# zhupan007/Detection_3D

Measured on AMD Instinct MI355X. Metric: buildings/sec inference, 4c_fpn432, higher is better.
Workload: dtype f32

## Files before the change

### detection_3d_amd/_lib.py

```python
import ctypes
import os

import torch

_HERE = os.path.dirname(os.path.abspath(__file__))
LIB_PATH = os.environ.get("D3D_LIB_PATH") or os.path.join(_HERE, "lib", "libd3d_hip.so")

_lib = None

c_int_p = ctypes.POINTER(ctypes.c_int)
c_float_p = ctypes.POINTER(ctypes.c_float)
vp = ctypes.c_void_p


class BnPrologue(ctypes.Structure):
    _fields_ = [("mean", vp), ("invstd", vp), ("weight", vp), ("bias", vp), ("leakiness", ctypes.c_float),
                ("out_stats", vp), ("out_stats_cap", ctypes.c_int), ("out_stats_rows", ctypes.POINTER(ctypes.c_int))]


bn_p = ctypes.POINTER(BnPrologue)

_SIGS = {
    "d3d_last_error": (ctypes.c_char_p, []),
    "d3d_abi_version": (ctypes.c_int, []),
    "d3d_meta_create": (ctypes.c_int, [ctypes.POINTER(vp), ctypes.c_size_t]),
    "d3d_meta_destroy": (ctypes.c_int, [vp]),
    "d3d_meta_clear": (ctypes.c_int, [vp]),
    "d3d_meta_arena_used": (ctypes.c_int, [vp, ctypes.POINTER(ctypes.c_size_t)]),
    "d3d_meta_set_geometry_stream": (ctypes.c_int, [vp, vp, ctypes.c_int]),
    "d3d_meta_set_plan_stream": (ctypes.c_int, [vp, vp, ctypes.c_int]),
    "d3d_geometry_async_start": (ctypes.c_int, [vp, vp, ctypes.c_int, vp, vp]),
    "d3d_geometry_async_wait": (ctypes.c_int, [vp, ctypes.c_int, ctypes.POINTER(ctypes.c_int), vp]),
    "d3d_geometry_async_finish": (ctypes.c_int, [vp]),
    "d3d_grid_chain_enable": (ctypes.c_int, [ctypes.c_int]),
    "d3d_conv_ws_mode": (ctypes.c_int, [ctypes.c_int]),
    "d3d_conv_late_mode": (ctypes.c_int, [ctypes.c_int]),
    "d3d_conv_dw_deterministic": (ctypes.c_int, [ctypes.c_int]),
    "d3d_conv_dw_thread_mode": (ctypes.c_int, [ctypes.c_int, vp, ctypes.c_size_t]),
    "d3d_conv_dw_scratch_bytes": (ctypes.c_size_t, [ctypes.c_int, ctypes.c_int, ctypes.c_int]),
    "d3d_grid_chain_head": (ctypes.c_int, [ctypes.c_int]),
    "d3d_sort_scratch_bytes": (ctypes.c_size_t, [ctypes.c_int, ctypes.c_int]),
    "d3d_sort_pairs": (ctypes.c_int, [vp, vp, ctypes.c_int, ctypes.c_int, ctypes.c_int, vp, vp, vp, ctypes.c_size_t, vp]),
    "d3d_conv_time_next": (ctypes.c_int, [vp, vp]),
    "d3d_input_layer_prepare": (ctypes.c_int, [vp, vp]),
    "d3d_post_scores": (ctypes.c_int, [vp, ctypes.c_int, ctypes.c_int, ctypes.c_float, vp, vp, vp]),
    "d3d_post_order": (ctypes.c_int, [vp, ctypes.c_int, ctypes.c_int, vp, vp]),
    "d3d_post_gather": (ctypes.c_int, [vp, vp, ctypes.c_int, ctypes.c_int, vp, vp, vp, vp]),
    "d3d_post_select_max": (ctypes.c_int, []),
    "d3d_post_select": (ctypes.c_int, [vp, vp, ctypes.c_int, ctypes.c_int, vp, vp, ctypes.c_int, ctypes.c_int, vp, vp, vp, vp,
                                       vp]),
    "d3d_roi_prepare": (ctypes.c_int, [vp, ctypes.c_int, ctypes.c_float, c_float_p, ctypes.c_int, ctypes.c_float, vp, vp,
                                       vp, vp]),
    "d3d_roi_prepare_counted": (ctypes.c_int, [vp, ctypes.c_int, vp, ctypes.c_float, c_float_p, ctypes.c_int,
                                               ctypes.c_float, vp, vp, vp, vp]),
    "d3d_voxelize": (ctypes.c_int, [vp, ctypes.c_int, ctypes.c_int, ctypes.c_double, c_int_p, vp, vp,
                                    c_int_p, vp, ctypes.c_size_t, vp]),
    "d3d_voxelize_scratch_bytes": (ctypes.c_size_t, [ctypes.c_int]),
    "d3d_input_layer_build": (ctypes.c_int, [vp, vp, ctypes.c_int, ctypes.c_int, c_int_p, ctypes.c_int,
                                             ctypes.c_int, vp, c_int_p]),
    "d3d_input_layer_build_prefetch": (ctypes.c_int, [vp, vp, ctypes.c_int, ctypes.c_int, c_int_p, ctypes.c_int,
                                                      ctypes.c_int, c_int_p, vp, c_int_p]),
    "d3d_input_layer_forward": (ctypes.c_int, [vp, vp, ctypes.c_int, vp, vp]),
    "d3d_input_layer_export": (ctypes.c_int, [vp, vp, vp, vp]),
    "d3d_get_n_active": (ctypes.c_int, [vp, c_int_p, c_int_p]),
    "d3d_get_spatial_locations": (ctypes.c_int, [vp, c_int_p, vp, vp]),
    "d3d_subm_prepare": (ctypes.c_int, [vp, c_int_p, c_int_p, vp, ctypes.POINTER(ctypes.c_long)]),
    "d3d_conv_prepare": (ctypes.c_int, [vp, c_int_p, c_int_p, c_int_p, c_int_p, vp, c_int_p,
                                        ctypes.POINTER(ctypes.c_long)]),
    "d3d_deconv_prepare": (ctypes.c_int, [vp, c_int_p, c_int_p, c_int_p, c_int_p, vp,
                                          ctypes.POINTER(ctypes.c_long)]),
    "d3d_export_rules": (ctypes.c_int, [vp, ctypes.c_int, c_int_p, c_int_p, c_int_p, vp, ctypes.c_long,
                                        ctypes.POINTER(ctypes.c_long), vp]),
    "d3d_packed_weight_floats": (ctypes.c_size_t, [ctypes.c_int, ctypes.c_int, ctypes.c_int]),
    "d3d_pack_conv_weight": (ctypes.c_int, [vp, ctypes.c_int, ctypes.c_int, ctypes.c_int, vp, vp]),
    "d3d_subm_conv_forward": (ctypes.c_int, [vp, c_int_p, c_int_p, vp, ctypes.c_int, vp, ctypes.c_int, vp,
                                             vp, vp, ctypes.POINTER(ctypes.c_double), bn_p]),
    "d3d_conv_forward": (ctypes.c_int, [vp, c_int_p, c_int_p, c_int_p, c_int_p, vp, ctypes.c_int, vp,
                                        ctypes.c_int, vp, vp, ctypes.POINTER(ctypes.c_double), bn_p]),
    "d3d_deconv_forward": (ctypes.c_int, [vp, c_int_p, c_int_p, c_int_p, c_int_p, vp, ctypes.c_int, vp,
                                          ctypes.c_int, vp, vp, vp, ctypes.POINTER(ctypes.c_double), bn_p]),
    "d3d_bn_apply": (ctypes.c_int, [vp, vp, ctypes.c_int, ctypes.c_int, vp, vp, vp, vp, ctypes.c_float, vp]),
    "d3d_bn_batch_invstd": (ctypes.c_int, [vp, ctypes.c_int, ctypes.c_int, ctypes.c_float, vp, vp, vp,
                                           ctypes.c_size_t, vp]),
    "d3d_pack_conv_weight_transposed": (ctypes.c_int, [vp, ctypes.c_int, ctypes.c_int, ctypes.c_int, ctypes.c_int,
                                                       vp, vp]),
    "d3d_subm_conv_backward": (ctypes.c_int, [vp, c_int_p, c_int_p, vp, ctypes.c_int, vp, ctypes.c_int, vp, vp,
                                              vp, vp]),
    "d3d_conv_backward": (ctypes.c_int, [vp, c_int_p, c_int_p, c_int_p, c_int_p, vp, ctypes.c_int, vp,
                                         ctypes.c_int, vp, vp, vp, vp]),
    "d3d_deconv_backward": (ctypes.c_int, [vp, c_int_p, c_int_p, c_int_p, c_int_p, vp, ctypes.c_int, vp,
                                           ctypes.c_int, vp, vp, vp, vp]),
    "d3d_bn_backward": (ctypes.c_int, [vp, vp, vp, vp, ctypes.c_int, ctypes.c_int, vp, vp, vp, vp, vp,
                                       ctypes.c_float, vp, ctypes.c_size_t, vp]),
    "d3d_bn_backward_scratch_bytes": (ctypes.c_size_t, [ctypes.c_int]),
    "d3d_input_layer_backward": (ctypes.c_int, [vp, vp, ctypes.c_int, vp, vp]),
    "d3d_sparse_to_dense_backward": (ctypes.c_int, [vp, c_int_p, vp, ctypes.c_int, vp, vp]),
    "d3d_roi_align_rotated_3d_backward": (ctypes.c_int, [vp, ctypes.c_int, ctypes.c_int, ctypes.c_int, ctypes.c_int,
                                                         ctypes.c_int, vp, ctypes.c_int, ctypes.c_float,
                                                         ctypes.c_int, ctypes.c_int, ctypes.c_int, ctypes.c_int,
                                                         vp, vp]),
    "d3d_roi_align_rotated_3d_sparse_backward": (ctypes.c_int, [vp, c_int_p, vp, ctypes.c_int, c_int_p, vp,
                                                                ctypes.c_int, ctypes.c_float, ctypes.c_int,
                                                                ctypes.c_int, ctypes.c_int, ctypes.c_int,
                                                                vp, vp]),
    "d3d_roi_align_rotated_3d_sparse_backward_deterministic": (
        ctypes.c_int, [vp, c_int_p, vp, ctypes.c_int, c_int_p, vp, ctypes.c_int, ctypes.c_float, ctypes.c_int,
                       ctypes.c_int, ctypes.c_int, ctypes.c_int, vp, ctypes.c_int, vp, ctypes.c_size_t, vp]),
    "d3d_roi_align_rotated_3d_sparse_backward_deterministic_scratch_bytes": (
        ctypes.c_size_t, [ctypes.c_int, ctypes.c_int, ctypes.c_int, ctypes.c_int, ctypes.c_int, ctypes.c_int,
                          ctypes.c_int]),
    "d3d_bn_forward": (ctypes.c_int, [vp, vp, ctypes.c_int, ctypes.c_int, vp, vp, vp, vp, vp, vp,
                                      ctypes.c_float, ctypes.c_float, ctypes.c_int, ctypes.c_float, vp,
                                      ctypes.c_size_t, vp]),
    "d3d_bn_batch_stats": (ctypes.c_int, [vp, ctypes.c_int, ctypes.c_int, vp, vp, vp, ctypes.c_size_t, vp]),
    "d3d_bn_scratch_bytes": (ctypes.c_size_t, [ctypes.c_int]),
    "d3d_add": (ctypes.c_int, [vp, vp, vp, ctypes.c_size_t, vp]),
    "d3d_sparse_to_dense_forward": (ctypes.c_int, [vp, c_int_p, vp, ctypes.c_int, ctypes.c_int, vp, vp]),
    "d3d_roi_align_rotated_3d_forward": (ctypes.c_int, [vp, ctypes.c_int, ctypes.c_int, ctypes.c_int,
                                                        ctypes.c_int, ctypes.c_int, vp, ctypes.c_int,
                                                        ctypes.c_float, ctypes.c_int, ctypes.c_int,
                                                        ctypes.c_int, ctypes.c_int, vp, vp]),
    "d3d_roi_align_rotated_3d_sparse_forward": (ctypes.c_int, [vp, c_int_p, vp, ctypes.c_int, c_int_p, vp,
                                                               ctypes.c_int, ctypes.c_float, ctypes.c_int,
                                                               ctypes.c_int, ctypes.c_int, ctypes.c_int,
                                                               vp, ctypes.c_int, ctypes.c_int, vp, vp]),
    "d3d_roi_align_rotated_3d_sparse_forward_levels": (ctypes.c_int, [vp, ctypes.c_int, c_int_p, ctypes.POINTER(vp),
                                                                      ctypes.c_int, c_float_p, vp, ctypes.c_int,
                                                                      ctypes.c_int, ctypes.c_int, ctypes.c_int,
                                                                      ctypes.c_int, vp, ctypes.c_int, vp, vp]),
    "d3d_rotate_iou_eval": (ctypes.c_int, [vp, ctypes.c_int, vp, ctypes.c_int, ctypes.c_int, vp, vp]),
    "d3d_boxes_iou_3d": (ctypes.c_int, [vp, ctypes.c_int, vp, ctypes.c_int, ctypes.POINTER(ctypes.c_float),
                                        ctypes.c_int, ctypes.c_int, vp, vp]),
    "d3d_match_segments": (ctypes.c_int, [vp, c_int_p, ctypes.c_int, vp, ctypes.c_int, vp, ctypes.POINTER(ctypes.c_float),
                                          ctypes.c_int, ctypes.c_float, ctypes.c_float, ctypes.c_float, ctypes.c_int,
                                          ctypes.POINTER(ctypes.c_float), vp, vp, vp, ctypes.c_size_t, vp]),
    "d3d_match_segments_scratch_bytes": (ctypes.c_size_t, [ctypes.c_int, ctypes.c_int]),
    "d3d_rotate_nms_3d_batched": (ctypes.c_int, [vp, vp, ctypes.c_int, vp, ctypes.c_int, ctypes.c_int, ctypes.c_float,
                                                 ctypes.c_float, ctypes.c_float, ctypes.c_int, vp, vp, vp,
                                                 ctypes.c_size_t, vp]),
    "d3d_nms_batched_scratch_bytes": (ctypes.c_size_t, [ctypes.c_int, ctypes.c_int]),
    "d3d_rotate_nms_3d": (ctypes.c_int, [vp, vp, ctypes.c_int, ctypes.c_int, ctypes.c_int, ctypes.c_float, ctypes.c_float,
                                         ctypes.c_float, vp, vp, c_int_p, vp, ctypes.c_size_t, vp]),
    "d3d_rotate_nms_3d_scratch_bytes": (ctypes.c_size_t, [ctypes.c_int, ctypes.c_int]),
    "d3d_topk_segments": (ctypes.c_int, [vp, ctypes.c_int, ctypes.c_int, ctypes.c_int, ctypes.c_int, vp, ctypes.c_int,
                                         ctypes.c_int, ctypes.c_int, c_float_p, c_int_p, vp, ctypes.c_int, vp,
                                         ctypes.c_float, vp, vp, vp, vp, vp, vp, ctypes.c_size_t, vp]),
    "d3d_topk_scratch_bytes": (ctypes.c_size_t, [ctypes.c_int, ctypes.c_int]),
    "d3d_topk_max": (ctypes.c_int, []),
    "d3d_anchors": (ctypes.c_int, [vp, c_int_p, ctypes.POINTER(ctypes.c_float), ctypes.c_int,
                                   ctypes.POINTER(ctypes.c_float), ctypes.c_float, vp, vp]),
    "d3d_anchors_maps": (ctypes.c_int, [vp, ctypes.c_int, c_int_p, ctypes.POINTER(ctypes.c_float), ctypes.c_int,
                                        ctypes.POINTER(ctypes.c_float), ctypes.c_float, vp, vp]),
    "d3d_rpn_head": (ctypes.c_int, [ctypes.POINTER(vp), c_int_p, ctypes.c_int, ctypes.c_int, vp, vp, vp, vp,
                                    ctypes.c_int, vp, vp, vp]),
    "d3d_mlp_heads": (ctypes.c_int, [vp, ctypes.c_int, ctypes.c_int, ctypes.c_int, vp, vp, vp, vp, vp, ctypes.c_int, vp, vp, vp]),
    "d3d_rotate_nms_3d_sorted": (ctypes.c_int, [vp, ctypes.c_int, ctypes.c_float, ctypes.c_int, vp, vp, vp,
                                                ctypes.c_size_t, vp]),
    "d3d_nms_scratch_bytes": (ctypes.c_size_t, [ctypes.c_int]),
    "d3d_box_decode": (ctypes.c_int, [vp, vp, ctypes.c_int, ctypes.POINTER(ctypes.c_float), ctypes.c_float,
                                      vp, vp]),
    "d3d_box_decode_classes": (ctypes.c_int, [vp, vp, ctypes.c_int, ctypes.c_int, ctypes.POINTER(ctypes.c_float),
                                              ctypes.c_float, vp, vp]),
    "d3d_box_decode_rows": (ctypes.c_int, [vp, vp, vp, ctypes.c_int, ctypes.POINTER(ctypes.c_float), ctypes.c_float,
                                           vp, vp]),
    "d3d_gather_kept": (ctypes.c_int, [vp, vp, vp, vp, ctypes.c_int, ctypes.c_float, vp, vp, vp, vp]),
    "d3d_plan_stats": (ctypes.c_int, [vp, ctypes.c_int, c_int_p, c_int_p, c_int_p, ctypes.POINTER(ctypes.c_long),
                                      ctypes.POINTER(ctypes.c_long), ctypes.POINTER(ctypes.c_long), vp]),
    "d3d_packed_weight_bytes": (ctypes.c_size_t, [ctypes.c_int, ctypes.c_int, ctypes.c_int, ctypes.c_int]),
    "d3d_pack_conv_weight_dt": (ctypes.c_int, [vp, ctypes.c_int, ctypes.c_int, ctypes.c_int, vp, ctypes.c_int, vp]),
    "d3d_subm_conv_forward_dt": (ctypes.c_int, [vp, c_int_p, c_int_p, vp, ctypes.c_int, vp, ctypes.c_int, vp, vp,
                                                ctypes.c_int, vp, ctypes.POINTER(ctypes.c_double), bn_p]),
    "d3d_conv_forward_dt": (ctypes.c_int, [vp, c_int_p, c_int_p, c_int_p, c_int_p, vp, ctypes.c_int, vp, ctypes.c_int,
                                           vp, ctypes.c_int, vp, ctypes.POINTER(ctypes.c_double), bn_p]),
    "d3d_deconv_forward_dt": (ctypes.c_int, [vp, c_int_p, c_int_p, c_int_p, c_int_p, vp, ctypes.c_int, vp, ctypes.c_int,
                                             vp, vp, ctypes.c_int, vp, ctypes.POINTER(ctypes.c_double), bn_p]),
    "d3d_conv_bf16_tuning": (ctypes.c_int, [ctypes.c_int, ctypes.c_long]),
    "d3d_bn_stats_from_partials": (ctypes.c_int, [vp, ctypes.c_int, ctypes.c_int, ctypes.c_int, ctypes.c_float, ctypes.c_int,
                                                  vp, vp, vp, ctypes.c_size_t, vp]),
    "d3d_bn_batch_invstd_dt": (ctypes.c_int, [vp, ctypes.c_int, ctypes.c_int, ctypes.c_float, vp, vp, vp,
                                              ctypes.c_size_t, ctypes.c_int, vp]),
    "d3d_rows_to_bf16": (ctypes.c_int, [vp, ctypes.c_long, ctypes.c_int, ctypes.c_int, vp, vp]),
    "d3d_bn_apply_dt": (ctypes.c_int, [vp, vp, ctypes.c_int, ctypes.c_int, vp, vp, vp, vp, ctypes.c_float,
                                       ctypes.c_int, vp]),
    "d3d_pack_conv_weight_transposed_dt": (ctypes.c_int, [vp, ctypes.c_int, ctypes.c_int, ctypes.c_int, ctypes.c_int,
                                                          vp, ctypes.c_int, vp]),
    "d3d_subm_conv_backward_dt": (ctypes.c_int, [vp, c_int_p, c_int_p, vp, ctypes.c_int, ctypes.c_int, vp, ctypes.c_int,
                                                 vp, vp, vp, ctypes.c_int, vp]),
    "d3d_conv_backward_dt": (ctypes.c_int, [vp, c_int_p, c_int_p, c_int_p, c_int_p, vp, ctypes.c_int, ctypes.c_int, vp,
                                            ctypes.c_int, vp, vp, vp, ctypes.c_int, vp]),
# ... 122 lines not shown
```

### detection_3d_amd/csrc/conv.hip

```cpp
#include <algorithm>

#include "d3d_internal.h"

namespace d3d {

typedef float f32x16 __attribute__((ext_vector_type(16)));
typedef float f32x4 __attribute__((ext_vector_type(4)));

__device__ __forceinline__ void wave_lds_sync() {
  __builtin_amdgcn_fence(__ATOMIC_RELEASE, "wavefront");
  __builtin_amdgcn_wave_barrier();
  __builtin_amdgcn_fence(__ATOMIC_ACQUIRE, "wavefront");
}

static inline int padded_cin(int cin) {
  if (cin <= 16) return 16;
  if (cin <= 32) return 32;
  if (cin <= 64) return 64;
  if (cin <= 128) return 128;
  if (cin <= 256) return 256;
  return -1;
}

__global__ void k_pack_weight(const float *__restrict__ w, int fv, int cin, int cout, int cp,
                              float *__restrict__ packed) {
  long t = (long)blockIdx.x * blockDim.x + threadIdx.x;
  long total = (long)fv * cp * cout;
  if (t >= total) return;
  int j = (int)(t & 3);
  long u = t >> 2;
  int co = (int)(u % cout);
  u /= cout;
  int g = (int)(u % (cp / 4));
  int k = (int)(u / (cp / 4));
  int ci = 4 * g + j;
  packed[t] = ci < cin ? w[((size_t)k * cin + ci) * cout + co] : 0.f;
}

template <int CT, int NCT, int COUT, int NT, int BPW, bool VEC, bool LATE = false>
__global__ __launch_bounds__(BPW *(COUT / 32 / NT) * 64) void k_conv(
    const float *__restrict__ in, int cin, const float *__restrict__ wp,
    const int32_t *__restrict__ nbrT, int npos, const int32_t *__restrict__ rows,
    const uint32_t *__restrict__ blkmask, int n_blk, const float *__restrict__ residual,
    float *__restrict__ out, int n_split, float *__restrict__ partial, BnPre pre, uint32_t in_bytes,
    double *__restrict__ stat) {
  constexpr int WPBLK = COUT / 32 / NT;
  static_assert(WPBLK == 1 || BPW == 1, "row blocks sharing a workgroup must be single-wave");
  constexpr int TPB = WPBLK * 64;
  constexpr int LDA = CT + 4;
  constexpr int CP = CT * NCT;
  constexpr int LPR = CT / 4;
  constexpr int RPP = TPB / LPR;
  constexpr int NIT = (32 / RPP) > 0 ? (32 / RPP) : 1;
  constexpr int NQ = CT / 8;
#ifndef D3D_QA
#define D3D_QA 8
#endif
  constexpr int QA = NQ < D3D_QA ? NQ : D3D_QA;
  static_assert(NQ % QA == 0, "ring depth must divide the q-iterations of a step");
  __shared__ __attribute__((aligned(16))) float smem[BPW * 32 * LDA];

  const int slot = threadIdx.x / TPB, tib = threadIdx.x % TPB;
  const int blk = blockIdx.x * BPW + slot;
  if (blk >= n_blk) return;
  float *As = smem + slot * 32 * LDA;
  const int lane = tib & 63, wib = tib >> 6;
  const int r = lane & 31, h = lane >> 5;
  const int grow = tib / LPR, gc4 = tib % LPR;
  const int colbase = wib * NT * 32;

  auto block_sync = [&]() {
    if constexpr (WPBLK == 1)
      wave_lds_sync();
    else
      __syncthreads();
  };

  uint32_t mask = __builtin_amdgcn_readfirstlane(blkmask[blk]);
  if (n_split > 1) {
    uint32_t keep = 0;
    for (uint32_t m = mask; m; m &= m - 1) {
      const int kk = __builtin_ctz(m);
      if (kk % n_split == (int)blockIdx.y) keep |= 1u << kk;
    }
    mask = keep;
  }
  const int rowid = rows[blk * 32 + r];
  f32x16 acc[NT];
#pragma unroll
  for (int nt = 0; nt < NT; nt++)
#pragma unroll
    for (int i = 0; i < 16; i++) acc[nt][i] = 0.f;

  const int32_t *nb = nbrT + (size_t)blk * 32;
  int idx[NIT];
  f32x4 stage[NIT];
  float mreal[NIT];
  int stage_ct = 0;
  f32x4 bnw[NCT], bnb[NCT];
#pragma unroll
  for (int t = 0; t < NCT; t++) {
    bnw[t] = {1.f, 1.f, 1.f, 1.f};
    bnb[t] = {0.f, 0.f, 0.f, 0.f};
    if (pre.mean) {
      const int c = t * CT + gc4 * 4;
      const f32x4 is = *(const f32x4 *)(pre.invstd + c), mu = *(const f32x4 *)(pre.mean + c);
      const f32x4 one = {1.f, 1.f, 1.f, 1.f}, zero = {0.f, 0.f, 0.f, 0.f};
      const f32x4 ga = pre.weight ? *(const f32x4 *)(pre.weight + c) : one;
      const f32x4 be = pre.bias ? *(const f32x4 *)(pre.bias + c) : zero;
      bnw[t] = is * ga;
      bnb[t] = -mu * bnw[t] + be;
    }
  }
  const uint32_t lane_piece = (uint32_t)gc4 * 16u, lane_idx = (uint32_t)grow * 4u;
  const __amdgpu_buffer_rsrc_t in_rsrc = __builtin_amdgcn_make_buffer_rsrc((void *)in, 0, (int)in_bytes, 0x00020000);
  auto load_idx = [&](int k) {
    const char *kb = (const char *)(nb + (size_t)k * npos);
#pragma unroll
    for (int it = 0; it < NIT; it++) {
      if constexpr (RPP <= 32) {
        idx[it] = *(const int32_t *)(kb + (lane_idx + (uint32_t)(it * RPP * 4)));
      } else {
        idx[it] = grow < 32 ? *(const int32_t *)(kb + lane_idx) : -1;
      }
    }
  };
  auto issue_data = [&](int ct) {
    stage_ct = ct;
#pragma unroll
    for (int it = 0; it < NIT; it++) {
      const int s = idx[it];
      mreal[it] = s >= 0 ? 1.f : 0.f;
      if constexpr (VEC) {
        const uint32_t off = s < 0 ? 0xfffffff0u : (uint32_t)s * (uint32_t)(CP * 4) + (uint32_t)(ct * CT * 4) + lane_piece;
        stage[it] = __builtin_bit_cast(f32x4, __builtin_amdgcn_raw_buffer_load_b128(in_rsrc, (int)off, 0, 0));
      } else {
        const float *p = in + (size_t)(s < 0 ? 0 : s) * cin + ct * CT + gc4 * 4;
        const int c = ct * CT + gc4 * 4;
        f32x4 v = {0.f, 0.f, 0.f, 0.f};
        if (c + 0 < cin) v[0] = p[0];
        if (c + 1 < cin) v[1] = p[1];
        if (c + 2 < cin) v[2] = p[2];
        if (c + 3 < cin) v[3] = p[3];
        stage[it] = v;
      }
    }
  };
  auto commit_gather = [&]() {
    const f32x4 bw = stage_ct == 0 ? bnw[0] : bnw[NCT - 1], bb = stage_ct == 0 ? bnb[0] : bnb[NCT - 1];
#pragma unroll
    for (int it = 0; it < NIT; it++) {
      const int row = it * RPP + grow;
      f32x4 v = stage[it];
      if constexpr (VEC) {
        if (pre.mean) v = bn_act(v, bw, bb, pre.leak) * mreal[it];
      } else {
        if (pre.mean) v = bn_act(v, bw, bb, pre.leak);
        const f32x4 zero = {0.f, 0.f, 0.f, 0.f};
        v = mreal[it] != 0.f ? v : zero;
      }
      if (row < 32) *(f32x4 *)(As + row * LDA + gc4 * 4) = v;
    }
  };

  auto next_k = [&](int k) -> int {
    const uint32_t m = k >= 31 ? 0u : (mask & ~((2u << k) - 1u));
    return m ? __builtin_ctz(m) : -1;
  };
  int k = mask ? __builtin_ctz(mask) : -1;
  int ct = 0;
  f32x4 ring[QA][NT];
  const uint32_t lane_b = (uint32_t)(h * COUT + r) * 16u;
  if (k >= 0) {
    load_idx(k);
    issue_data(0);
    const int k_after = NCT > 1 ? k : next_k(k);
    if (k_after >= 0 && k_after != k) load_idx(k_after);
    const char *wk0 = (const char *)(wp + ((size_t)(k * (CP / 4)) * COUT + colbase) * 4);
#pragma unroll
    for (int q = 0; q < QA; q++)
#pragma unroll
      for (int nt = 0; nt < NT; nt++)
        ring[q][nt] = *(const f32x4 *)(wk0 + (lane_b + (uint32_t)((2 * q * COUT + nt * 32) * 16)));
  }
  while (k >= 0) {
    commit_gather();
    block_sync();
    int nk = k, nct = ct + 1;
    if (nct == NCT) {
      nct = 0;
      nk = next_k(k);
    }
    const int k2 = nk < 0 ? -1 : ((nct + 1 < NCT) ? nk : next_k(nk));
    if constexpr (!LATE) {
      if (nk >= 0) {
        issue_data(nct);
        if (k2 >= 0 && k2 != nk) load_idx(k2);
      }
    }
    __builtin_amdgcn_s_setprio(1);
    const char *wk = (const char *)(wp + ((size_t)(k * (CP / 4) + ct * (CT / 4)) * COUT + colbase) * 4);
    const char *wk_next = nk >= 0 ? (const char *)(wp + ((size_t)(nk * (CP / 4) + nct * (CT / 4)) * COUT + colbase) * 4) : wk;
#pragma unroll
    for (int q = 0; q < NQ; q++) {
      f32x4 b[NT];
#pragma unroll
      for (int nt = 0; nt < NT; nt++) b[nt] = ring[q % QA][nt];
      {
        const char *src = (q + QA < NQ) ? wk : wk_next;
        const int qq = (q + QA) % NQ;
#pragma unroll
        for (int nt = 0; nt < NT; nt++)
          ring[q % QA][nt] = *(const f32x4 *)(src + (lane_b + (uint32_t)((2 * qq * COUT + nt * 32) * 16)));
      }
      const f32x4 a = *(const f32x4 *)(As + r * LDA + q * 8 + h * 4);
#pragma unroll
      for (int nt = 0; nt < NT; nt++) {
        acc[nt] = __builtin_amdgcn_mfma_f32_32x32x2f32(a[0], b[nt][0], acc[nt], 0, 0, 0);
        acc[nt] = __builtin_amdgcn_mfma_f32_32x32x2f32(a[1], b[nt][1], acc[nt], 0, 0, 0);
        acc[nt] = __builtin_amdgcn_mfma_f32_32x32x2f32(a[2], b[nt][2], acc[nt], 0, 0, 0);
        acc[nt] = __builtin_amdgcn_mfma_f32_32x32x2f32(a[3], b[nt][3], acc[nt], 0, 0, 0);
      }
      if constexpr (LATE) {
        if (q == 0) {
          if (nk < 0) {
#pragma unroll
            for (int it = 0; it < NIT; it++) idx[it] = -1;
          }
          issue_data(nk >= 0 ? nct : 0);
          load_idx(k2 >= 0 ? k2 : k);
        }
      }
    }
    if constexpr (!LATE) {
      __builtin_amdgcn_sched_group_barrier(0x020, 2 * NIT, 0);
      __builtin_amdgcn_sched_group_barrier(0x100, 1, 0);
#pragma unroll
      for (int q = 0; q < NQ; q++) {
        __builtin_amdgcn_sched_group_barrier(0x008, 1, 0);
        __builtin_amdgcn_sched_group_barrier(0x100, 1, 0);
        __builtin_amdgcn_sched_group_barrier(0x020, NT, 0);
        __builtin_amdgcn_sched_group_barrier(0x008, 4 * NT - 1, 0);
      }
    } else {
      __builtin_amdgcn_sched_group_barrier(0x100, 1, 0);
#pragma unroll
      for (int q = 0; q < NQ; q++) {
        __builtin_amdgcn_sched_group_barrier(0x008, 1, 0);
        __builtin_amdgcn_sched_group_barrier(0x100, 1, 0);
        __builtin_amdgcn_sched_group_barrier(0x020, NT, 0);
        __builtin_amdgcn_sched_group_barrier(0x008, 4 * NT - 1, 0);
        if (q == 0) __builtin_amdgcn_sched_group_barrier(0x020, 2 * NIT, 0);
      }
    }
    __builtin_amdgcn_s_setprio(0);
    block_sync();
    k = nk;
    ct = nct;
  }
  if (n_split > 1) {
    float *pt = partial + ((size_t)blockIdx.y * npos + (size_t)blk * 32) * COUT;
#pragma unroll
    for (int reg = 0; reg < 16; reg++) {
      const int row_in = (reg & 3) + 8 * (reg >> 2) + 4 * h;
#pragma unroll
      for (int nt = 0; nt < NT; nt++) pt[(size_t)row_in * COUT + colbase + nt * 32 + r] = acc[nt][reg];
    }
    return;
  }
  double cs[NT], css[NT];
#pragma unroll
  for (int nt = 0; nt < NT; nt++) cs[nt] = css[nt] = 0.0;
#pragma unroll
  for (int g4 = 0; g4 < 4; g4++) {
    int orow[4];
    float res[4][NT];
#pragma unroll
    for (int j = 0; j < 4; j++) orow[j] = __shfl(rowid, j + 8 * g4 + 4 * h, 64);
    if (residual) {
#pragma unroll
      for (int j = 0; j < 4; j++)
#pragma unroll
        for (int nt = 0; nt < NT; nt++)
          res[j][nt] = residual[(size_t)(orow[j] < 0 ? 0 : orow[j]) * COUT + colbase + nt * 32 + r];
#pragma unroll
      for (int j = 0; j < 4; j++)
#pragma unroll
        for (int nt = 0; nt < NT; nt++) acc[nt][g4 * 4 + j] += res[j][nt];
    }
#pragma unroll
    for (int j = 0; j < 4; j++) {
      if (orow[j] < 0) continue;
#pragma unroll
      for (int nt = 0; nt < NT; nt++) out[(size_t)orow[j] * COUT + colbase + nt * 32 + r] = acc[nt][g4 * 4 + j];
      if (stat) {
#pragma unroll
        for (int nt = 0; nt < NT; nt++) {
          const double d = (double)acc[nt][g4 * 4 + j];
          cs[nt] += d;
          css[nt] += d * d;
        }
      }
    }
  }
  if (stat) {
    double *sp = stat + (size_t)blk * (2 * COUT);
#pragma unroll
    for (int nt = 0; nt < NT; nt++) {
      const double a = cs[nt] + __shfl_xor(cs[nt], 32, 64), b = css[nt] + __shfl_xor(css[nt], 32, 64);
      if (h == 0) {
        sp[colbase + nt * 32 + r] = a;
        sp[COUT + colbase + nt * 32 + r] = b;
      }
    }
  }
}

__global__ __launch_bounds__(256) void k_conv_reduce(const float *__restrict__ partial, int n_split,
                                                     int npos, int cout4, const int32_t *__restrict__ rows,
                                                     const float *__restrict__ residual,
                                                     float *__restrict__ out, double *__restrict__ stat) {
  __shared__ double red[2][256][4];
  const long t = (long)blockIdx.x * blockDim.x + threadIdx.x;
  const bool in_range = t < (long)npos * cout4;
  const int pos = in_range ? (int)(t / cout4) : 0, c4 = (int)(t % cout4);
  const int orow = in_range ? rows[pos] : -1;
  f32x4 acc = {0.f, 0.f, 0.f, 0.f};
  if (orow >= 0) {
    for (int y = 0; y < n_split; y++) acc += *(const f32x4 *)(partial + (((size_t)y * npos + pos) * cout4 + c4) * 4);
    const size_t o = ((size_t)orow * cout4 + c4) * 4;
    if (residual) acc += *(const f32x4 *)(residual + o);
    *(f32x4 *)(out + o) = acc;
  }
  if (!stat) return;
#pragma unroll
  for (int j = 0; j < 4; j++) {
    const double d = orow >= 0 ? (double)acc[j] : 0.0;
    red[0][threadIdx.x][j] = d;
    red[1][threadIdx.x][j] = d * d;
  }
  __syncthreads();
  if ((int)threadIdx.x < cout4) {
    double *sp = stat + (size_t)blockIdx.x * (8 * cout4);
#pragma unroll
    for (int j = 0; j < 4; j++) {
      double a = 0.0, b = 0.0;
      for (int q = threadIdx.x; q < 256; q += cout4) {
        a += red[0][q][j];
        b += red[1][q][j];
      }
      sp[c4 * 4 + j] = a;
      sp[4 * cout4 + c4 * 4 + j] = b;
    }
  }
}

static constexpr int kSplitTargetWaves = 4096;
static bool g_conv_late = [] {
  const char *e = getenv("D3D_CONV_LATE");
  return !(e && e[0] == '0');
}();

static thread_local hipEvent_t t_time_start = nullptr, t_time_stop = nullptr;
void conv_timing_take(hipEvent_t *start, hipEvent_t *stop) {
  *start = t_time_start;
  *stop = t_time_stop;
  t_time_start = t_time_stop = nullptr;
}

struct StatOut {
  double *buf;
  int cap;
  int *rows_host;
};

template <int CT, int NCT, int COUT, int NT, int BPW>
static int launch_t(d3d_meta *m, const Plan &p, const float *in, int cin, const float *wp,
                    const float *residual, float *out, hipStream_t s, BnPre pre, const StatOut &so) {
  constexpr int WPBLK = COUT / 32 / NT;
  constexpr int threads = BPW * WPBLK * 64;
  const int npos = p.n_blk * 32;
  const long waves = (long)p.n_blk * WPBLK;
  int n_split = 1;
  if (BPW == 1 && p.K > 1 && m) {
    if (waves < kSplitTargetWaves) n_split = (int)std::min<long>(p.K, (kSplitTargetWaves + waves - 1) / waves);
  }
  float *partial = nullptr;
  size_t mark = 0;
  if (n_split > 1) {
    mark = m->feat_arena.used;
    partial = m->feat_arena.get<float>((size_t)n_split * npos * COUT);
    if (!partial) n_split = 1;
  }
  const dim3 grid((p.n_blk + BPW - 1) / BPW, n_split);
  const long reduce_blocks = ((long)npos * (COUT / 4) + 255) / 256;
  const long stat_rows = n_split > 1 ? reduce_blocks : p.n_blk;
  double *stat = (so.buf && stat_rows <= so.cap) ? so.buf : nullptr;
  if (so.rows_host) *so.rows_host = stat ? (int)stat_rows : 0;
  const uint32_t in_bytes = (uint32_t)((size_t)p.n_in * (size_t)cin * 4);
  const hipEvent_t ev_start = t_time_start, ev_stop = t_time_stop;
  t_time_start = t_time_stop = nullptr;
  if (ev_start) (void)hipEventRecord(ev_start, s);
  if (cin == CT * NCT && n_split == 1 && launch_conv_ws(p, in, cin, wp, COUT, residual, out, s, pre, stat, in_bytes)) {
  } else if (cin == CT * NCT && g_conv_late && CT >= 32)
    hipLaunchKernelGGL((k_conv<CT, NCT, COUT, NT, BPW, true, true>), grid, dim3(threads), 0, s, in, cin, wp, p.nbrT, npos,
                       p.rows, p.blkmask, p.n_blk, residual, out, n_split, partial, pre, in_bytes,
                       n_split > 1 ? nullptr : stat);
  else if (cin == CT * NCT)
    hipLaunchKernelGGL((k_conv<CT, NCT, COUT, NT, BPW, true>), grid, dim3(threads), 0, s, in, cin, wp, p.nbrT, npos,
                       p.rows, p.blkmask, p.n_blk, residual, out, n_split, partial, pre, in_bytes,
                       n_split > 1 ? nullptr : stat);
  else
    hipLaunchKernelGGL((k_conv<CT, NCT, COUT, NT, BPW, false>), grid, dim3(threads), 0, s, in, cin, wp, p.nbrT, npos,
                       p.rows, p.blkmask, p.n_blk, residual, out, n_split, partial, pre, in_bytes,
                       n_split > 1 ? nullptr : stat);
  if (ev_stop) (void)hipEventRecord(ev_stop, s);
  if (n_split > 1) {
    const long total = (long)npos * (COUT / 4);
    hipLaunchKernelGGL(k_conv_reduce, dim3((unsigned)((total + 255) / 256)), dim3(256), 0, s, partial, n_split,
                       npos, COUT / 4, p.rows, residual, out, stat);
    m->feat_arena.used = mark;
  }
  D3D_LAUNCH_CHECK();
  return D3D_OK;
}

template <int CT, int NCT>
static int launch_c(d3d_meta *m, const Plan &p, const float *in, int cin, const float *wp, int cout,
                    const float *residual, float *out, hipStream_t s, BnPre pre, const StatOut &so) {
  switch (cout) {
    case 32: return launch_t<CT, NCT, 32, 1, 4>(m, p, in, cin, wp, residual, out, s, pre, so);
    case 64: return launch_t<CT, NCT, 64, 1, 1>(m, p, in, cin, wp, residual, out, s, pre, so);
    case 128: return launch_t<CT, NCT, 128, 1, 1>(m, p, in, cin, wp, residual, out, s, pre, so);
    case 256: return launch_t<CT, NCT, 256, 1, 1>(m, p, in, cin, wp, residual, out, s, pre, so);
  }
  set_error("convolution: Cout=%d not supported (32, 64, 128, 256)", cout);
  return D3D_ERR_UNSUPPORTED;
}

int launch_conv(d3d_meta *m, const Plan &p, const float *in, int cin, const float *packed_w, int cout,
                const float *residual, float *out, hipStream_t s, const d3d_bn_prologue *bn) {
  if (bn && bn->out_stats_rows) *bn->out_stats_rows = 0;
  if (p.n_rows == 0) {
    if (t_time_start) (void)hipEventRecord(t_time_start, s);
    if (t_time_stop) (void)hipEventRecord(t_time_stop, s);
    t_time_start = t_time_stop = nullptr;
    return D3D_OK;
  }
  D3D_REQUIRE(in && packed_w && out, "convolution: null pointer");
  D3D_REQUIRE((size_t)p.n_in * (size_t)cin * 4 < ((size_t)1 << 32),
              "convolution: gathered tensor of %d rows x %d channels exceeds the 4 GiB of the 32-bit gather offsets", p.n_in, cin);
  BnPre pre = {nullptr, nullptr, nullptr, nullptr, 0.f};
  StatOut so = {nullptr, 0, nullptr};
  if (bn) {
    so = {bn->out_stats, bn->out_stats_cap, bn->out_stats_rows};
    if (so.rows_host) *so.rows_host = 0;
  }
  if (bn && bn->mean) {
    D3D_REQUIRE(bn->invstd && cin % 8 == 0 && padded_cin(cin) == cin, "fused BatchNorm prologue needs Cin in {32,64,128,256}");
    pre = {bn->mean, bn->invstd, bn->weight, bn->bias, bn->leakiness};
  }
  switch (padded_cin(cin)) {
    case 16: return launch_c<16, 1>(m, p, in, cin, packed_w, cout, residual, out, s, pre, so);
    case 32: return launch_c<32, 1>(m, p, in, cin, packed_w, cout, residual, out, s, pre, so);
    case 64: return launch_c<64, 1>(m, p, in, cin, packed_w, cout, residual, out, s, pre, so);
    case 128: return launch_c<128, 1>(m, p, in, cin, packed_w, cout, residual, out, s, pre, so);
    case 256: return launch_c<128, 2>(m, p, in, cin, packed_w, cout, residual, out, s, pre, so);
  }
  set_error("convolution: Cin=%d not supported (<= 256)", cin);
  return D3D_ERR_UNSUPPORTED;
}

}

using namespace d3d;

extern "C" {

int d3d_conv_late_mode(int on) {
  const int was = g_conv_late ? 1 : 0;
  if (on >= 0) g_conv_late = on != 0;
  return was;
}

int d3d_conv_time_next(void *start_event, void *stop_event) {
  t_time_start = (hipEvent_t)start_event;
  t_time_stop = (hipEvent_t)stop_event;
  return D3D_OK;
}

size_t d3d_packed_weight_floats(int fv, int cin, int cout) {
  int cp = padded_cin(cin);
  if (cp < 0 || fv <= 0 || cout <= 0) return 0;
  return (size_t)fv * cp * cout;
}

int d3d_pack_conv_weight(const float *w, int fv, int cin, int cout, float *packed, void *stream) {
  hipStream_t s = (hipStream_t)stream;
  int cp = padded_cin(cin);
  D3D_REQUIRE(w && packed && fv > 0 && cout > 0 && cp > 0, "pack_conv_weight: bad arguments (Cin=%d)", cin);
  long total = (long)fv * cp * cout;
  hipLaunchKernelGGL(k_pack_weight, dim3((unsigned)((total + 255) / 256)), dim3(256), 0, s, w, fv, cin, cout, cp, packed);
  D3D_LAUNCH_CHECK();
  return D3D_OK;
}

int d3d_subm_conv_forward(d3d_meta *m, const int *size, const int *filt, const float *in, int cin,
                          const float *packed_w, int cout, const float *residual, float *out,
                          void *stream, double *macs_host, const d3d_bn_prologue *bn) {
  hipStream_t s = (hipStream_t)stream;
  D3D_REQUIRE(m && size && filt, "null argument");
  int rc = d3d_subm_prepare(m, size, filt, stream, nullptr);
  if (rc) return rc;
  Plan *p = const_cast<Plan *>(find_plan(m, 0, size, filt, nullptr));
  if (macs_host) {
    long nr;
    rc = plan_rules(m, *p, s, &nr);
    if (rc) return rc;
    *macs_host = (double)nr * cin * cout;
  }
  return launch_conv(m, *p, in, cin, packed_w, cout, residual, out, s, bn);
}

int d3d_conv_forward(d3d_meta *m, const int *in_size, const int *out_size, const int *filt,
                     const int *stride, const float *in, int cin, const float *packed_w, int cout,
                     float *out, void *stream, double *macs_host, const d3d_bn_prologue *bn) {
  hipStream_t s = (hipStream_t)stream;
  D3D_REQUIRE(m && in_size && out_size && filt && stride, "null argument");
  int rc = d3d_conv_prepare(m, in_size, out_size, filt, stride, stream, nullptr, nullptr);
  if (rc) return rc;
  Plan *p = const_cast<Plan *>(find_plan(m, 1, in_size, filt, stride));
  if (macs_host) {
    long nr;
    rc = plan_rules(m, *p, s, &nr);
    if (rc) return rc;
    *macs_host = (double)nr * cin * cout;
  }
  return launch_conv(m, *p, in, cin, packed_w, cout, nullptr, out, s, bn);
}

int d3d_deconv_forward(d3d_meta *m, const int *in_size, const int *out_size, const int *filt,
                       const int *stride, const float *in, int cin, const float *packed_w, int cout,
                       const float *residual, float *out, void *stream, double *macs_host,
                       const d3d_bn_prologue *bn) {
  hipStream_t s = (hipStream_t)stream;
  D3D_REQUIRE(m && in_size && out_size && filt && stride, "null argument");
  const Plan *p = nullptr;
  int rc = get_deconv_plan(m, out_size, filt, stride, s, &p);
  if (rc) return rc;
  if (macs_host) {
    long nr;
    rc = plan_rules(m, *const_cast<Plan *>(p), s, &nr);
    if (rc) return rc;
    *macs_host = (double)nr * cin * cout;
  }
  return launch_conv(m, *p, in, cin, packed_w, cout, residual, out, s, bn);
}

int d3d_subm_conv_forward_dt(d3d_meta *m, const int *size, const int *filt, const void *in, int cin,
                             const void *packed_w, int cout, const void *residual, void *out, int dtype, void *stream,
                             double *macs_host, const d3d_bn_prologue *bn) {
  if (dtype == D3D_F32)
    return d3d_subm_conv_forward(m, size, filt, (const float *)in, cin, (const float *)packed_w, cout,
                                 (const float *)residual, (float *)out, stream, macs_host, bn);
  hipStream_t s = (hipStream_t)stream;
  D3D_REQUIRE(dtype == D3D_BF16 && m && size && filt, "subm_conv_forward_dt: bad arguments");
  int rc = d3d_subm_prepare(m, size, filt, stream, nullptr);
  if (rc) return rc;
  Plan *p = const_cast<Plan *>(find_plan(m, 0, size, filt, nullptr));
  if (macs_host) {
    long nr;
    rc = plan_rules(m, *p, s, &nr);
    if (rc) return rc;
    *macs_host = (double)nr * cin * cout;
  }
  return launch_conv_bf16(m, *p, in, cin, packed_w, cout, residual, out, s, bn);
}

int d3d_conv_forward_dt(d3d_meta *m, const int *in_size, const int *out_size, const int *filt, const int *stride,
                        const void *in, int cin, const void *packed_w, int cout, void *out, int dtype, void *stream,
                        double *macs_host, const d3d_bn_prologue *bn) {
  if (dtype == D3D_F32)
    return d3d_conv_forward(m, in_size, out_size, filt, stride, (const float *)in, cin, (const float *)packed_w, cout,
                            (float *)out, stream, macs_host, bn);
  hipStream_t s = (hipStream_t)stream;
  D3D_REQUIRE(dtype == D3D_BF16 && m && in_size && out_size && filt && stride, "conv_forward_dt: bad arguments");
  int rc = d3d_conv_prepare(m, in_size, out_size, filt, stride, stream, nullptr, nullptr);
  if (rc) return rc;
  Plan *p = const_cast<Plan *>(find_plan(m, 1, in_size, filt, stride));
  if (macs_host) {
    long nr;
    rc = plan_rules(m, *p, s, &nr);
    if (rc) return rc;
    *macs_host = (double)nr * cin * cout;
  }
  return launch_conv_bf16(m, *p, in, cin, packed_w, cout, nullptr, out, s, bn);
}

int d3d_deconv_forward_dt(d3d_meta *m, const int *in_size, const int *out_size, const int *filt, const int *stride,
                          const void *in, int cin, const void *packed_w, int cout, const void *residual, void *out,
                          int dtype, void *stream, double *macs_host, const d3d_bn_prologue *bn) {
  if (dtype == D3D_F32)
    return d3d_deconv_forward(m, in_size, out_size, filt, stride, (const float *)in, cin, (const float *)packed_w, cout,
                              (const float *)residual, (float *)out, stream, macs_host, bn);
  hipStream_t s = (hipStream_t)stream;
  D3D_REQUIRE(dtype == D3D_BF16 && m && in_size && out_size && filt && stride, "deconv_forward_dt: bad arguments");
  const Plan *p = nullptr;
  int rc = get_deconv_plan(m, out_size, filt, stride, s, &p);
  if (rc) return rc;
  if (macs_host) {
    long nr;
    rc = plan_rules(m, *const_cast<Plan *>(p), s, &nr);
    if (rc) return rc;
    *macs_host = (double)nr * cin * cout;
  }
  return launch_conv_bf16(m, *p, in, cin, packed_w, cout, residual, out, s, bn);
}

}
```

### include/d3d_hip.h

```cpp
#ifndef D3D_HIP_H
#define D3D_HIP_H
#include <stddef.h>
#include <stdint.h>

#ifdef __cplusplus
extern "C" {
#endif

typedef enum {
  D3D_OK = 0,
  D3D_ERR_ARG = -1,
  D3D_ERR_HIP = -2,
  D3D_ERR_NOMEM = -3,
  D3D_ERR_STATE = -4,
  D3D_ERR_UNSUPPORTED = -5
} d3d_status;

const char *d3d_last_error(void);
int d3d_abi_version(void);

typedef struct d3d_meta d3d_meta;
int d3d_meta_create(d3d_meta **out, size_t arena_bytes);
int d3d_meta_destroy(d3d_meta *m);
int d3d_meta_clear(d3d_meta *m);
int d3d_meta_arena_used(d3d_meta *m, size_t *bytes_host);
int d3d_meta_set_geometry_stream(d3d_meta *m, void *stream, int enable);
int d3d_grid_chain_enable(int on);
int d3d_conv_ws_mode(int mode);
int d3d_conv_late_mode(int on);
int d3d_grid_chain_head(int levels);
int d3d_geometry_async_start(d3d_meta *m, const int *specs_host, int n, void *stream, void *view_stream);
int d3d_geometry_async_wait(d3d_meta *m, int index, int *n_out_host, void *wait_stream);
int d3d_geometry_async_finish(d3d_meta *m);
int d3d_meta_set_plan_stream(d3d_meta *m, void *stream, int enable);

size_t d3d_sort_scratch_bytes(int n, int bits);
int d3d_sort_pairs(const uint32_t *keys, const int32_t *vals, int n, int bits, int descending, uint32_t *keys_out,
                   int32_t *vals_out, void *scratch, size_t scratch_bytes, void *stream);

int d3d_voxelize(const float *pcl, int n, int nfeat, double scale, const int *full_scale_host,
                 int64_t *coords_out, float *feats_out, int *n_kept_host, void *scratch,
                 size_t scratch_bytes, void *stream);
size_t d3d_voxelize_scratch_bytes(int n);

int d3d_input_layer_build(d3d_meta *m, const int64_t *coords, int n, int ncols,
                          const int *spatial_size_host, int batch_size, int mode, void *stream,
                          int *n_active_host);
int d3d_input_layer_build_prefetch(d3d_meta *m, const int64_t *coords, int n, int ncols,
                                   const int *spatial_size_host, int batch_size, int mode,
                                   const int *prefetch_filter_host, void *stream, int *n_active_host);
int d3d_input_layer_prepare(d3d_meta *m, void *stream);
int d3d_input_layer_forward(d3d_meta *m, const float *feats, int planes, float *out, void *stream);
int d3d_input_layer_export(d3d_meta *m, int32_t *offsets, int32_t *idx, void *stream);

int d3d_get_n_active(d3d_meta *m, const int *spatial_size_host, int *n_host);
int d3d_get_spatial_locations(d3d_meta *m, const int *spatial_size_host, int64_t *out, void *stream);

int d3d_anchors(d3d_meta *m, const int *spatial_size_host, const float *base_host, int A,
                const float *stride_host, float voxel_scale, float *out, void *stream);
int d3d_anchors_maps(d3d_meta *m, int n_maps, const int *sizes_host, const float *bases_host, int A,
                     const float *strides_host, float voxel_scale, float *out, void *stream);

#define D3D_RPN_MAX_MAPS 6
int d3d_rpn_head(const float *const *maps_host, const int *rows_host, int n_maps, int channels,
                 const float *w1_packed, const float *b1, const float *w2_packed, const float *b2, int a,
                 float *objectness, float *regression, void *stream);
int d3d_mlp_heads(const float *x, int rows, int channels, int relu_in, const float *w1_packed, const float *b1,
                  float *t_out, const float *w2_packed, const float *b2, int a, float *out_a, float *out_7a, void *stream);

int d3d_subm_prepare(d3d_meta *m, const int *spatial_size_host, const int *filter_host,
                     void *stream, long *n_rules_host);
int d3d_conv_prepare(d3d_meta *m, const int *in_size_host, const int *out_size_host,
                     const int *filter_host, const int *stride_host, void *stream,
                     int *n_out_host, long *n_rules_host);
int d3d_deconv_prepare(d3d_meta *m, const int *in_size_host, const int *out_size_host,
                       const int *filter_host, const int *stride_host, void *stream,
                       long *n_rules_host);
int d3d_export_rules(d3d_meta *m, int kind, const int *in_size_host, const int *filter_host,
                     const int *stride_host, int32_t *triples, long capacity, long *n_host,
                     void *stream);

int d3d_plan_stats(d3d_meta *m, int kind, const int *in_size_host, const int *filter_host, const int *stride_host,
                   long *n_blocks_host, long *executed_host, long *rules_host, void *stream);

int d3d_conv_time_next(void *start_event, void *stop_event);
size_t d3d_packed_weight_floats(int filter_volume, int cin, int cout);
int d3d_pack_conv_weight(const float *w, int filter_volume, int cin, int cout, float *packed,
                         void *stream);

typedef struct {
  const float *mean, *invstd, *weight, *bias;
  float leakiness;
  double *out_stats;
  int out_stats_cap;
  int *out_stats_rows;
} d3d_bn_prologue;
int d3d_subm_conv_forward(d3d_meta *m, const int *spatial_size_host, const int *filter_host,
                          const float *in, int cin, const float *packed_w, int cout,
                          const float *residual, float *out, void *stream, double *macs_host,
                          const d3d_bn_prologue *bn_host);
int d3d_conv_forward(d3d_meta *m, const int *in_size_host, const int *out_size_host,
                     const int *filter_host, const int *stride_host, const float *in, int cin,
                     const float *packed_w, int cout, float *out, void *stream, double *macs_host,
                     const d3d_bn_prologue *bn_host);
int d3d_deconv_forward(d3d_meta *m, const int *in_size_host, const int *out_size_host,
                       const int *filter_host, const int *stride_host, const float *in, int cin,
                       const float *packed_w, int cout, const float *residual, float *out,
                       void *stream, double *macs_host, const d3d_bn_prologue *bn_host);

typedef enum { D3D_F32 = 0, D3D_BF16 = 1 } d3d_dtype;
size_t d3d_packed_weight_bytes(int filter_volume, int cin, int cout, int dtype);
int d3d_pack_conv_weight_dt(const float *w, int filter_volume, int cin, int cout, void *packed, int dtype,
                            void *stream);
int d3d_subm_conv_forward_dt(d3d_meta *m, const int *spatial_size_host, const int *filter_host, const void *in,
                             int cin, const void *packed_w, int cout, const void *residual, void *out, int dtype,
                             void *stream, double *macs_host, const d3d_bn_prologue *bn_host);
int d3d_conv_forward_dt(d3d_meta *m, const int *in_size_host, const int *out_size_host, const int *filter_host,
                        const int *stride_host, const void *in, int cin, const void *packed_w, int cout, void *out,
                        int dtype, void *stream, double *macs_host, const d3d_bn_prologue *bn_host);
int d3d_deconv_forward_dt(d3d_meta *m, const int *in_size_host, const int *out_size_host, const int *filter_host,
                          const int *stride_host, const void *in, int cin, const void *packed_w, int cout,
                          const void *residual, void *out, int dtype, void *stream, double *macs_host,
                          const d3d_bn_prologue *bn_host);
int d3d_conv_bf16_tuning(int row_blocks, long min_waves);
int d3d_bn_stats_from_partials(const double *partials, int partial_rows, int rows, int planes, float eps,
                               int want_invstd, float *mean, float *var_or_invstd, void *scratch, size_t scratch_bytes,
                               void *stream);
int d3d_bn_batch_invstd_dt(const void *in, int rows, int planes, float eps, float *mean, float *invstd,
                           void *scratch, size_t scratch_bytes, int dtype, void *stream);
int d3d_bn_apply_dt(const void *in, void *out, int rows, int planes, const float *mean, const float *invstd,
                    const float *weight, const float *bias, float leakiness, int dtype, void *stream);
int d3d_rows_to_bf16(const float *in, long rows, int cin, int width, void *out, void *stream);

int d3d_pack_conv_weight_transposed(const float *w, int filter_volume, int cin, int cout, int flip,
                                    float *packed, void *stream);
int d3d_subm_conv_backward(d3d_meta *m, const int *spatial_size_host, const int *filter_host,
                           const float *in, int cin, const float *packed_wt_flipped, int cout,
                           const float *d_out, float *d_in, float *d_weight, void *stream);
int d3d_conv_backward(d3d_meta *m, const int *in_size_host, const int *out_size_host,
                      const int *filter_host, const int *stride_host, const float *in, int cin,
                      const float *packed_wt, int cout, const float *d_out, float *d_in,
                      float *d_weight, void *stream);
int d3d_deconv_backward(d3d_meta *m, const int *in_size_host, const int *out_size_host,
                        const int *filter_host, const int *stride_host, const float *in, int cin,
                        const float *packed_wt, int cout, const float *d_out, float *d_in,
                        float *d_weight, void *stream);
int d3d_pack_conv_weight_transposed_dt(const float *w, int filter_volume, int cin, int cout, int flip, void *packed,
                                       int dtype, void *stream);
int d3d_subm_conv_backward_dt(d3d_meta *m, const int *spatial_size_host, const int *filter_host, const void *in,
                              int cs, int cin, const void *packed_wt_flipped, int cout, const void *d_out, void *d_in,
                              float *d_weight, int dtype, void *stream);
int d3d_conv_backward_dt(d3d_meta *m, const int *in_size_host, const int *out_size_host, const int *filter_host,
                         const int *stride_host, const void *in, int cs, int cin, const void *packed_wt, int cout,
                         const void *d_out, void *d_in, float *d_weight, int dtype, void *stream);
int d3d_deconv_backward_dt(d3d_meta *m, const int *in_size_host, const int *out_size_host, const int *filter_host,
                           const int *stride_host, const void *in, int cs, int cin, const void *packed_wt, int cout,
                           const void *d_out, void *d_in, float *d_weight, int dtype, void *stream);
int d3d_conv_dw_deterministic(int on);
int d3d_conv_dw_thread_mode(int on, void *scratch, size_t scratch_bytes);
size_t d3d_conv_dw_scratch_bytes(int filter_volume, int cin, int cout);
int d3d_bn_backward(const float *in, const float *out, const float *d_out, float *d_in, int rows,
                    int planes, const float *save_mean, const float *save_invstd, const float *weight,
                    float *d_weight, float *d_bias, float leakiness, void *scratch,
                    size_t scratch_bytes, void *stream);
size_t d3d_bn_backward_scratch_bytes(int planes);
int d3d_bn_backward_dt(const void *in, const void *out, const void *d_out, void *d_in, int rows, int planes,
                       const float *save_mean, const float *save_invstd, const float *weight, float *d_weight,
                       float *d_bias, float leakiness, void *scratch, size_t scratch_bytes, int dtype, void *stream);
int d3d_input_layer_backward(d3d_meta *m, const float *d_out, int planes, float *d_in, void *stream);
int d3d_sparse_to_dense_backward(d3d_meta *m, const int *spatial_size_host, const float *d_out, int planes,
                                 float *d_in, void *stream);
int d3d_roi_align_rotated_3d_backward(const float *top_diff, int B, int C, int H, int W, int Z,
                                      const float *rois, int K, float spatial_scale, int ph, int pw,
                                      int pz, int sampling_ratio, float *bottom_diff, void *stream);
int d3d_roi_align_rotated_3d_sparse_backward(d3d_meta *m, const int *spatial_size_host,
                                             const float *top_diff, int C, const int *crop_host,
                                             const float *rois, int K, float spatial_scale, int ph,
                                             int pw, int pz, int sampling_ratio, float *d_feats,
                                             void *stream);
int d3d_roi_align_rotated_3d_sparse_backward_deterministic(d3d_meta *m, const int *spatial_size_host,
                                                           const float *top_diff, int C, const int *crop_host,
                                                           const float *rois, int K, float spatial_scale, int ph,
// ... 95 lines not shown
```

Baseline: 212.2.

## Reduce split-K conv partials inside the workgroup instead of a separate reduce kernel

Adds a slice-group variant of the sparse conv kernel in which several waves of one workgroup each handle a residue class of kernel offsets for the same row block. Their accumulators are summed in LDS and the result is written with residual and BN statistics directly. This removes the global partial buffer and the follow-up k_conv_reduce launch when the split fits in the configured number of rounds. The cost is fewer workgroups, extra LDS, and block-wide barriers, with idle waves syncing when their residue has fewer steps.

```diff
diff --git a/detection_3d_amd/_lib.py b/detection_3d_amd/_lib.py
--- a/detection_3d_amd/_lib.py
+++ b/detection_3d_amd/_lib.py
@@ -35,6 +35,7 @@
     "d3d_grid_chain_enable": (ctypes.c_int, [ctypes.c_int]),
     "d3d_conv_ws_mode": (ctypes.c_int, [ctypes.c_int]),
     "d3d_conv_late_mode": (ctypes.c_int, [ctypes.c_int]),
+    "d3d_conv_split_rounds": (ctypes.c_int, [ctypes.c_int]),
     "d3d_conv_dw_deterministic": (ctypes.c_int, [ctypes.c_int]),
     "d3d_conv_dw_thread_mode": (ctypes.c_int, [ctypes.c_int, vp, ctypes.c_size_t]),
     "d3d_conv_dw_scratch_bytes": (ctypes.c_size_t, [ctypes.c_int, ctypes.c_int, ctypes.c_int]),
diff --git a/detection_3d_amd/csrc/conv.hip b/detection_3d_amd/csrc/conv.hip
--- a/detection_3d_amd/csrc/conv.hip
+++ b/detection_3d_amd/csrc/conv.hip
@@ -37,8 +37,8 @@
   packed[t] = ci < cin ? w[((size_t)k * cin + ci) * cout + co] : 0.f;
 }
 
-template <int CT, int NCT, int COUT, int NT, int BPW, bool VEC, bool LATE = false>
-__global__ __launch_bounds__(BPW *(COUT / 32 / NT) * 64) void k_conv(
+template <int CT, int NCT, int COUT, int NT, int BPW, bool VEC, bool LATE = false, int G = 1>
+__global__ __launch_bounds__(G *BPW *(COUT / 32 / NT) * 64) void k_conv(
     const float *__restrict__ in, int cin, const float *__restrict__ wp,
     const int32_t *__restrict__ nbrT, int npos, const int32_t *__restrict__ rows,
     const uint32_t *__restrict__ blkmask, int n_blk, const float *__restrict__ residual,
@@ -58,10 +58,13 @@
 #endif
   constexpr int QA = NQ < D3D_QA ? NQ : D3D_QA;
   static_assert(NQ % QA == 0, "ring depth must divide the q-iterations of a step");
-  __shared__ __attribute__((aligned(16))) float smem[BPW * 32 * LDA];
-
-  const int slot = threadIdx.x / TPB, tib = threadIdx.x % TPB;
-  const int blk = blockIdx.x * BPW + slot;
+  static_assert(G == 1 || BPW == 1, "slice groups share one row block");
+  constexpr int SMEM = (G * BPW * 32 * LDA > (G > 1 ? G * 32 * COUT : 0)) ? G * BPW * 32 * LDA : G * 32 * COUT;
+  __shared__ __attribute__((aligned(16))) float smem[SMEM + (G > 1 ? 32 * COUT : 0)];
+  float *osum = smem + SMEM;
+
+  const int slot = G > 1 ? __builtin_amdgcn_readfirstlane(threadIdx.x / TPB) : threadIdx.x / TPB, tib = threadIdx.x % TPB;
+  const int blk = G > 1 ? blockIdx.x : blockIdx.x * BPW + slot;
   if (blk >= n_blk) return;
   float *As = smem + slot * 32 * LDA;
   const int lane = tib & 63, wib = tib >> 6;
@@ -70,14 +73,15 @@
   const int colbase = wib * NT * 32;
 
   auto block_sync = [&]() {
-    if constexpr (WPBLK == 1)
+    if constexpr (WPBLK == 1 && G == 1)
       wave_lds_sync();
     else
       __syncthreads();
   };
 
-  uint32_t mask = __builtin_amdgcn_readfirstlane(blkmask[blk]);
-  if (n_split > 1) {
+  const uint32_t full = __builtin_amdgcn_readfirstlane(blkmask[blk]);
+  uint32_t mask = full;
+  if (G == 1 && n_split > 1) {
     uint32_t keep = 0;
     for (uint32_t m = mask; m; m &= m - 1) {
       const int kk = __builtin_ctz(m);
@@ -87,6 +91,25 @@
   }
   const int rowid = rows[blk * 32 + r];
   f32x16 acc[NT];
+
+  constexpr int NTH = G * TPB;
+  constexpr int E = G > 1 ? 32 * COUT / NTH : 1;
+  static_assert(G == 1 || E * NTH == 32 * COUT, "slice groups must cover the row block's tile evenly");
+  if constexpr (G > 1) {
+#pragma unroll
+    for (int i = 0; i < E; i++) osum[threadIdx.x + i * NTH] = 0.f;
+  }
+  auto residue_mask = [&](int y) -> uint32_t {
+    uint32_t sel = 0;
+    for (int kk = y; kk < 32; kk += n_split) sel |= 1u << kk;
+    return full & sel;
+  };
+  for (int y0 = 0; y0 < (G > 1 ? n_split : 1); y0 += G) {
+  int steps = 0;
+  if constexpr (G > 1) {
+    mask = y0 + slot < n_split ? residue_mask(y0 + slot) : 0u;
+    for (int g = 0; g < G && y0 + g < n_split; g++) steps = max(steps, __builtin_popcount(residue_mask(y0 + g)) * NCT);
+  }
 #pragma unroll
   for (int nt = 0; nt < NT; nt++)
 #pragma unroll
@@ -183,7 +206,12 @@
       for (int nt = 0; nt < NT; nt++)
         ring[q][nt] = *(const f32x4 *)(wk0 + (lane_b + (uint32_t)((2 * q * COUT + nt * 32) * 16)));
   }
-  while (k >= 0) {
+  while (G == 1 ? k >= 0 : steps-- > 0) {
+    if (G > 1 && k < 0) {
+      __syncthreads();
+      __syncthreads();
+      continue;
+    }
     commit_gather();
     block_sync();
     int nk = k, nct = ct + 1;
@@ -257,6 +285,56 @@
     block_sync();
     k = nk;
     ct = nct;
+  }
+  if constexpr (G > 1) {
+    float *pt = smem + slot * 32 * COUT;
+#pragma unroll
+    for (int reg = 0; reg < 16; reg++) {
+      const int row_in = (reg & 3) + 8 * (reg >> 2) + 4 * h;
+#pragma unroll
+      for (int nt = 0; nt < NT; nt++) pt[row_in * COUT + colbase + nt * 32 + r] = acc[nt][reg];
+    }
+    __syncthreads();
+#pragma unroll
+    for (int i = 0; i < E; i++) {
+      const int e = threadIdx.x + i * NTH;
+      float v = osum[e];
+      for (int g = 0; g < G && y0 + g < n_split; g++) v += smem[g * 32 * COUT + e];
+      osum[e] = v;
+    }
+    __syncthreads();
+  }
+  }
+  if constexpr (G > 1) {
+#pragma unroll
+    for (int i = 0; i < E; i++) {
+      const int e = threadIdx.x + i * NTH, row = e / COUT, col = e % COUT;
+      const int orow = rows[blk * 32 + row];
+      float v = osum[e];
+      if (orow >= 0) {
+        if (residual) v += residual[(size_t)orow * COUT + col];
+        out[(size_t)orow * COUT + col] = v;
+      }
+      smem[e] = v;
+    }
+    if (stat) {
+      constexpr int R = 1024 / COUT;
+      __syncthreads();
+      for (int t = threadIdx.x; t < (COUT / 32) * COUT; t += NTH) {
+        const int v = t / COUT, c = t % COUT;
+        double a = 0.0, b = 0.0;
+        for (int rr = 0; rr < R; rr++) {
+          const int row = v * R + rr;
+          const double d = rows[blk * 32 + row] >= 0 ? (double)smem[row * COUT + c] : 0.0;
+          a += d;
+          b += d * d;
+        }
+        double *sp = stat + ((size_t)blk * (COUT / 32) + v) * (2 * COUT);
+        sp[c] = a;
+        sp[COUT + c] = b;
+      }
+    }
+    return;
   }
   if (n_split > 1) {
     float *pt = partial + ((size_t)blockIdx.y * npos + (size_t)blk * 32) * COUT;
@@ -356,6 +434,10 @@
 }
 
 static constexpr int kSplitTargetWaves = 4096;
+static int g_conv_split_rounds = [] {
+  const char *e = getenv("D3D_CONV_SPLIT_ROUNDS");
+  return e && e[0] ? atoi(e) : 1;
+}();
 static bool g_conv_late = [] {
   const char *e = getenv("D3D_CONV_LATE");
   return !(e && e[0] == '0');
@@ -385,9 +467,12 @@
   if (BPW == 1 && p.K > 1 && m) {
     if (waves < kSplitTargetWaves) n_split = (int)std::min<long>(p.K, (kSplitTargetWaves + waves - 1) / waves);
   }
+  constexpr int GS = (BPW == 1 && WPBLK <= 4) ? 8 / WPBLK : 1;
+  const bool in_wg = GS > 1 && n_split > 1 && cin == CT * NCT && g_conv_late && CT >= 32 &&
+                     (n_split + GS - 1) / GS <= g_conv_split_rounds;
   float *partial = nullptr;
   size_t mark = 0;
-  if (n_split > 1) {
+  if (n_split > 1 && !in_wg) {
     mark = m->feat_arena.used;
     partial = m->feat_arena.get<float>((size_t)n_split * npos * COUT);
     if (!partial) n_split = 1;
@@ -401,7 +486,11 @@
   const hipEvent_t ev_start = t_time_start, ev_stop = t_time_stop;
   t_time_start = t_time_stop = nullptr;
   if (ev_start) (void)hipEventRecord(ev_start, s);
-  if (cin == CT * NCT && n_split == 1 && launch_conv_ws(p, in, cin, wp, COUT, residual, out, s, pre, stat, in_bytes)) {
+  if (in_wg) {
+    if constexpr (GS > 1)
+      hipLaunchKernelGGL((k_conv<CT, NCT, COUT, NT, 1, true, true, GS>), dim3(p.n_blk), dim3(GS * threads), 0, s, in, cin,
+                         wp, p.nbrT, npos, p.rows, p.blkmask, p.n_blk, residual, out, n_split, nullptr, pre, in_bytes, stat);
+  } else if (cin == CT * NCT && n_split == 1 && launch_conv_ws(p, in, cin, wp, COUT, residual, out, s, pre, stat, in_bytes)) {
   } else if (cin == CT * NCT && g_conv_late && CT >= 32)
     hipLaunchKernelGGL((k_conv<CT, NCT, COUT, NT, BPW, true, true>), grid, dim3(threads), 0, s, in, cin, wp, p.nbrT, npos,
                        p.rows, p.blkmask, p.n_blk, residual, out, n_split, partial, pre, in_bytes,
@@ -415,7 +504,7 @@
                        p.rows, p.blkmask, p.n_blk, residual, out, n_split, partial, pre, in_bytes,
                        n_split > 1 ? nullptr : stat);
   if (ev_stop) (void)hipEventRecord(ev_stop, s);
-  if (n_split > 1) {
+  if (n_split > 1 && !in_wg) {
     const long total = (long)npos * (COUT / 4);
     hipLaunchKernelGGL(k_conv_reduce, dim3((unsigned)((total + 255) / 256)), dim3(256), 0, s, partial, n_split,
                        npos, COUT / 4, p.rows, residual, out, stat);
@@ -480,6 +569,12 @@
 int d3d_conv_late_mode(int on) {
   const int was = g_conv_late ? 1 : 0;
   if (on >= 0) g_conv_late = on != 0;
+  return was;
+}
+
+int d3d_conv_split_rounds(int rounds) {
+  const int was = g_conv_split_rounds;
+  if (rounds >= 0) g_conv_split_rounds = rounds;
   return was;
 }
 
diff --git a/include/d3d_hip.h b/include/d3d_hip.h
--- a/include/d3d_hip.h
+++ b/include/d3d_hip.h
@@ -28,6 +28,7 @@
 int d3d_grid_chain_enable(int on);
 int d3d_conv_ws_mode(int mode);
 int d3d_conv_late_mode(int on);
+int d3d_conv_split_rounds(int rounds);
 int d3d_grid_chain_head(int levels);
 int d3d_geometry_async_start(d3d_meta *m, const int *specs_host, int n, void *stream, void *view_stream);
 int d3d_geometry_async_wait(d3d_meta *m, int index, int *n_out_host, void *wait_stream);
```

New measurement: 212.5, median of 6. Within noise of the previous version (+0.1%).
